# yutiansut/marl-optimal-execution

Hardware: AMD Instinct MI355X
Metric: env-steps/sec (whole node), rmsc03 100-agent market ×4096 envs, 1/2/4/8 GPUs (higher is better)
Workload: dtype int64; 1 GPU; rmsc03 x4096 envs per GPU, full episode per step (config build from seeds + the config's session), seeds 123456789+global_env; envs_per_gpu=4096, global_envs=4096, parallelism=envs sharded, dp1, parity_hash=False, env_errors=0, agents_per_env=64, device=AMD Radeon Graphics, cus=256

## Files before the change

include/mxa.h:

```cpp
#ifndef MXA_H
#define MXA_H
#include <stdint.h>
#ifdef __cplusplus
extern "C" {
#endif

typedef struct mxa_handle mxa_handle;

enum { MXA_RMSC03 = 0, MXA_SPARSE_ZI_100 = 1, MXA_SPARSE_ZI_1000 = 2, MXA_MARKETREPLAY = 3, MXA_RMSC03_RL = 4,
       MXA_VALUE_NOISE = 5 ,
       MXA_RMSC01 = 6 ,
       MXA_RMSC02 = 7 ,
       MXA_OBI_RMSC02 = 8 ,
       MXA_RANDOM_FUND_VALUE = 9 ,
       MXA_RANDOM_FUND_DIVERSE = 10 ,
       MXA_HIST_FUND_VALUE = 11 ,
       MXA_HIST_FUND_DIVERSE = 12 ,
       MXA_MARKETREPLAY_RUNNER = 13 ,
       MXA_MARKETREPLAY_TWAP = 14 ,
       MXA_RMSC03_SBMM = 15, MXA_RMSC03_SBMM_POLL = 16,
       MXA_RMSC03_MM = 17 };
enum {
  MXA_OK = 0, MXA_EINVAL = -1, MXA_EHIP = -2, MXA_ENOMEM = -3, MXA_ERANGE = -4
};
// ... 83 lines not shown
int mxa_set_launch_schedule(mxa_handle* h, int64_t first_chunk);
int mxa_set_stop_time(mxa_handle* h, int64_t t_stop_ns);
int mxa_run_until(mxa_handle* h, int64_t t_stop_ns, int64_t* events_out);
int mxa_finalize(mxa_handle* h);
int mxa_read_final(mxa_handle* h, int32_t env, mxa_agent_final* out, int32_t cap);
int mxa_read_summary(mxa_handle* h, mxa_env_summary* out );
int mxa_read_agents(mxa_handle* h, int32_t env, mxa_agent_state* out, int32_t cap);
int mxa_read_book(mxa_handle* h, int32_t env, int32_t side, int64_t* out4, int32_t cap);
int mxa_read_trace(mxa_handle* h, int32_t env, int64_t* out , int64_t cap, int64_t* n);
int mxa_set_seeds(mxa_handle* h, const uint32_t* seeds);
int mxa_write_results(mxa_handle* h, void* device_out);
#define MXA_RECORD_WORDS 12
int mxa_write_records(mxa_handle* h, void* device_out);
#define MXA_COUNTER_WORDS 34
int mxa_read_counters(mxa_handle* h, int64_t* out);
#define MXA_INPLACE_WORDS 6
int mxa_read_inplace(mxa_handle* h, uint64_t* out);
int mxa_read_raw(mxa_handle* h, int32_t env, int64_t offset, int64_t bytes, void* out);
int mxa_layout(const mxa_handle* h, int64_t* offsets8);
int32_t mxa_n_agents(const mxa_handle* h);
int32_t mxa_n_envs(const mxa_handle* h);
int64_t mxa_env_bytes(const mxa_handle* h);
int mxa_set_stream(mxa_handle* h, void* stream);
double mxa_last_kernel_ms(const mxa_handle* h);
const char* mxa_last_error(const mxa_handle* h);
void mxa_destroy(mxa_handle* h);

int mxa_create_replay(const int64_t* t, const int64_t* oid, const int64_t* price, const int64_t* size,
                      const int8_t* buy, int32_t n_rec, int32_t n_envs, int32_t device, int32_t trace_cap,
                      mxa_handle** out);
int mxa_create_replay_runner(const int64_t* t, const int64_t* oid, const int64_t* price, const int64_t* size,
// ... 26 lines not shown
  int32_t price;
  int32_t qty;
} mxa_book_rec;
#define MXA_BL_FUNDAMENTAL (-2147483647 - 1)
int mxa_set_book_log(mxa_handle* h, int32_t cap);
#define MXA_BL_EV_RX (-2147483647 - 1 + 256)
#define MXA_BL_EV_NT (MXA_BL_EV_RX + 256)
#define MXA_BL_EV_PLACE (MXA_BL_EV_RX + 512)
#define MXA_BL_EV_END (MXA_BL_EV_RX + 768)
int mxa_set_exchange_log(mxa_handle* h, int32_t on);
int mxa_read_book_log(mxa_handle* h, int32_t env, mxa_book_rec* out, int64_t cap, int64_t* n);

#include "mxa_snap.h"
#include "mxa_depth.h"
#include "mxa_bars.h"

int mxa_rng_probe(int32_t device, uint32_t seed, int32_t mode, double a, double b, int32_t n, double* out);
int mxa_math_probe(int32_t device, int32_t mode, const double* x, const double* y, double* out, int64_t n);
int mxa_policy_probe(void* stream, int32_t n, const float* x, const float* params, int32_t n_layers,
                     const int32_t* dims, int32_t test, int32_t enough, const double* u, const int64_t* rnd,
                     const double* eps, float* q, int64_t* a);

#ifdef __cplusplus
}
#endif
#endif
```

marl-optimal-execution_amd/build_lib.py:

```python
import hashlib
import os
import subprocess
import sys
from concurrent.futures import ThreadPoolExecutor

HERE = os.path.dirname(os.path.abspath(__file__))
ROOT = os.path.dirname(HERE)
SRC = os.path.join(HERE, "csrc", "mxa_api.hip")
INST = os.path.join(HERE, "csrc", "mxa_inst.hip")
OUT = os.path.join(HERE, "lib", "libmxa.so")
OBJ = os.path.join(HERE, "build")
N_CONFIGS = 18
DEPS = ["mxa_api.hip", "mxa_inst.hip", "mxa_entry.h", "mxa_kernels.hip", "mxa_layout.h", "mxa_config.h", "glibc_math.h",
        "glibc_math_tables.h", "qnet_wave_device.h", "ddqn_device.h", "mxa_snapshot.h", "mxa_depth_kernels.h",
        "mxa_bars_kernels.h"]
HIPCC = os.environ.get("HIPCC", "/opt/rocm/bin/hipcc")
FLAGS = ["--offload-arch=gfx950", "-O3", "-std=c++20", "-ffp-contract=off", "-fno-fast-math", "-fPIC", "-shared",
         "-Wno-unused-result", "-Wno-unused-value", "-mllvm", "-structurizecfg-skip-uniform-regions"]

CFG_FLAGS = {1: ["-mllvm", "-amdgpu-sched-strategy=max-ilp"], 2: ["-fno-slp-vectorize"],
             3: ["-mllvm", "-amdgpu-sched-strategy=max-ilp"]}


def sources():
    return [os.path.join(HERE, "csrc", d) for d in DEPS] + [os.path.join(ROOT, "include", h) for h in ("mxa.h", "mxa_snap.h", "mxa_depth.h", "mxa_bars.h")]


def build_id(extra=()):
    h = hashlib.sha256()
    for s in sources():
        with open(s, "rb") as f:
            h.update(f.read())
    h.update(" ".join(FLAGS + list(extra)).encode())
    h.update(repr(sorted(CFG_FLAGS.items())).encode())
    return h.hexdigest()[:16]


def up_to_date():
    if not os.path.exists(OUT):
        return False
# ... 54 lines not shown
```

marl-optimal-execution_amd/csrc/mxa_api.hip:

```cpp
#include <hip/hip_runtime.h>

#include <dlfcn.h>
#include <spawn.h>
#include <sys/stat.h>
#include <sys/wait.h>
#include <unistd.h>

#include <algorithm>
#include <cstddef>
#include <cstdio>
#include <cstdlib>
#include <cstring>
#include <map>
#include <memory>
#include <mutex>
#include <string>
#include <vector>

extern char** environ;

#include "../../include/mxa.h"
#define MXA_API_TU
#include "mxa_kernels.hip"
#include "mxa_entry.h"
// ... 1216 lines not shown
  hipSetDevice(h->device);
  delete h;
}

int mxa_rng_probe(int32_t device, uint32_t seed, int32_t mode, double a, double b, int32_t n, double* out) {
  if (n <= 0 || !out || mode < 0 || mode > 5) return MXA_EINVAL;
  if (hipSetDevice(device) != hipSuccess) return MXA_EHIP;
  DevBuf<double> d_out;
  DevBuf<uint32_t> d_s;
  if (d_out.alloc(n) != hipSuccess || d_s.alloc(MXA_RNG_WORDS) != hipSuccess) return MXA_ENOMEM;
  hipLaunchKernelGGL(mxa_rng_probe_kernel, dim3(1), dim3(64), 0, 0, seed, mode, a, b, n, d_out.p, d_s.p);
  if (hipGetLastError() != hipSuccess) return MXA_EHIP;
  return hipMemcpy(out, d_out, sizeof(double) * n, hipMemcpyDeviceToHost) == hipSuccess ? MXA_OK : MXA_EHIP;
}

int mxa_math_probe(int32_t device, int32_t mode, const double* x, const double* y, double* out, int64_t n) {
  if (n <= 0 || !x || !out) return MXA_EINVAL;
  if (hipSetDevice(device) != hipSuccess) return MXA_EHIP;
  DevBuf<double> dx, dy, dout;
  size_t bytes = sizeof(double) * n;
  if (dx.alloc(n) != hipSuccess || dy.alloc(n) != hipSuccess || dout.alloc(n) != hipSuccess) return MXA_ENOMEM;
  if (hipMemcpy(dx, x, bytes, hipMemcpyHostToDevice) != hipSuccess ||
      hipMemcpy(dy, y ? y : x, bytes, hipMemcpyHostToDevice) != hipSuccess)
    return MXA_EHIP;
  hipLaunchKernelGGL(mxa_math_probe_kernel, dim3((unsigned)((n + 255) / 256)), dim3(256), 0, 0, mode, dx.p, dy.p, dout.p,
                     n);
  if (hipGetLastError() != hipSuccess) return MXA_EHIP;
  return hipMemcpy(out, dout, bytes, hipMemcpyDeviceToHost) == hipSuccess ? MXA_OK : MXA_EHIP;
}

// ... 237 lines not shown
```

marl-optimal-execution_amd/csrc/mxa_config.h:

```cpp
#pragma once
#include <stddef.h>
#include "mxa_layout.h"
#include "../../include/mxa.h"

namespace mxa_cfg {

constexpr int64_t NS = 1000000000LL;
constexpr int64_t MIN = 60 * NS;
constexpr int64_t HOUR = 60 * MIN;

struct Shape {
  int sq, so;
  bool pl;
  int waves;
  int pw;
  int hot;
  int sql = 0;
};
constexpr int sq_lds(int cfg);
constexpr int lat_lds(int cfg);
constexpr Shape shape(int cfg);
#ifndef MXA_RMSC03_WAVES
#define MXA_RMSC03_WAVES 4
#endif
#ifndef MXA_RMSC01_WAVES
#define MXA_RMSC01_WAVES 4
#endif
#ifndef MXA_W_RMSC02
#define MXA_W_RMSC02 2
#endif
#ifndef MXA_BOOK_LDS_RMSC02
#define MXA_BOOK_LDS_RMSC02 0x34
#endif
#ifndef MXA_PL_RMSC02
#define MXA_PL_RMSC02 1
#endif
// ... 97 lines not shown
#define MXA_BOOK_LDS_RFV 0x34
#endif
constexpr int book_lds(int cfg) {
  return cfg == MXA_CFG_RMSC02 ? MXA_BOOK_LDS_RMSC02
         : (cfg >= MXA_CFG_RANDOM_FUND_VALUE && cfg <= MXA_CFG_HIST_FUND_DIVERSE) ? MXA_BOOK_LDS_RFV
                                                                                 : 0;
}
#ifndef MXA_TEMPER_FILL_MASK
#define MXA_TEMPER_FILL_MASK ((1 << MXA_CFG_RMSC03) | (1 << MXA_CFG_SPARSE_ZI_100) | (1 << MXA_CFG_VALUE_NOISE))
#endif
#ifndef MXA_ONE_ADVANCE_MASK
#define MXA_ONE_ADVANCE_MASK MXA_TEMPER_FILL_MASK
#endif
constexpr bool temper_fill(int cfg) { return (((MXA_TEMPER_FILL_MASK) >> cfg) & 1) != 0; }
constexpr bool one_advance(int cfg) { return (((MXA_ONE_ADVANCE_MASK) >> cfg) & 1) != 0; }
constexpr size_t lds_bytes(int cfg) {
  return (size_t)sq_lds(cfg) * 64 * (12 + (shape(cfg).pl ? 4 * shape(cfg).pw : 0)) + 512
         + (size_t)shape(cfg).hot * 512
         + 1024
         + (size_t)lat_lds(cfg) * 8
         + (rp_hdr_lds(cfg) ? 256 : 0)
         + (size_t)__builtin_popcount(book_lds(cfg)) * shape(cfg).so * 256
         + 256
#ifdef MXA_PROF
         + 1024
#endif
      ;
}

constexpr void base_params(MxaParams& P) {
  P.o_rbar = 1e5;
  P.o_kappa = 1.67e-12;
  P.o_fundvol = 1e-4;
  P.o_lambda = 2.77778e-13;
// ... 349 lines not shown
  off = align_up(off + (uint64_t)L.qcap * sizeof(SavedEvent) + (S.pl ? 0 : (uint64_t)L.qcap * 4 * S.pw) +
                     (uint64_t)(S.sq - sq_lds(cfg)) * 64 * 12,
                 256);
  L.off_book = (uint32_t)off;
  off = align_up(off + (uint64_t)L.ocap * sizeof(SavedOrder), 256);
  L.off_tx = (uint32_t)off;
  off = align_up(off + 64 + (uint64_t)L.tx_cap * sizeof(TxRec), 256);
  L.off_oh = off;
  off = align_up(off + (uint64_t)L.oh_cap * sizeof(OhRec), 256);
  L.off_hh = off;
  off = align_up(off + (uint64_t)L.hbl_range * 8, 256);
  L.off_sub = off;
  off = align_up(off + (P.md_sub ? (uint64_t)MD_MAX_SUBS * sizeof(SubRec) : 0), 256);
  L.off_md = off;
  off = align_up(off + (P.md_sub ? (uint64_t)P.n_agents * MD_WORDS * 4 : 0), 256);
  L.off_trace = (uint32_t)off;
  L.env_stride = off;
}

constexpr void params_value_noise(MxaParams& P) {
  base_params(P);
  P.config = MXA_CFG_VALUE_NOISE;
  P.ex_log_orders = 0;
  P.mkt_close = 10 * HOUR + 30 * MIN;
  P.start = 0;
  P.stop = 17 * HOUR;
  P.default_comp_delay = 1000000000;
  P.lat_mode = 1;
  P.noise_len = 6;
  P.lat_lo = 21000;
// ... 324 lines not shown
```

marl-optimal-execution_amd/csrc/mxa_kernels.hip:

```cpp
#pragma once
#include <hip/hip_runtime.h>
#if defined(MXA_ONLY_RMSC03) && !(defined(MXA_ONLY_CFG) && (MXA_ONLY_CFG == 3 || MXA_ONLY_CFG == 4))
#define MXA_NO_GYM
#endif

#ifndef MXA_HINT_MASK
#define MXA_HINT_MASK ((1 << 0) | (1 << 4))
#endif
#ifndef MXA_HINT_GROUPS
#define MXA_HINT_GROUPS 3
#endif
#if defined(MXA_INST_CFG)
#define MXA_HINT_ON (((MXA_HINT_MASK) >> (MXA_INST_CFG)) & 1)
#elif defined(MXA_ONLY_RMSC03) && defined(MXA_ONLY_CFG)
#define MXA_HINT_ON (((MXA_HINT_MASK) >> (MXA_ONLY_CFG)) & 1)
#elif defined(MXA_ONLY_RMSC03)
#define MXA_HINT_ON ((MXA_HINT_MASK) & 1)
#else
#define MXA_HINT_ON 0
#endif
#define MXA_EXPECT_(x, v) __builtin_expect(!!(x), v)
#define MXA_PROB_(x, v, p) __builtin_expect_with_probability(!!(x), v, p)
#if MXA_HINT_ON && ((MXA_HINT_GROUPS) & 1)
#define MXA_LIKELY(x) MXA_EXPECT_(x, 1)
// ... 337 lines not shown
    x1 = 2.0 * rs_double(r) - 1.0;
    x2 = 2.0 * rs_double(r) - 1.0;
    r2 = x1 * x1 + x2 * x2;
  } while (MXA_RARE_P(r2 >= 1.0 || r2 == 0.0, 0.215));
  f = __builtin_sqrt(-2.0 * gm_log(r2) / r2);
  r.gauss = f * x1;
  r.hasg |= 1;
  return f * x2;
}
template <bool B, int W, bool TF>
DEV double rs_normal(RSt<B, W, TF>& r, double loc, double scale) { return loc + scale * rs_gauss(r); }
template <bool B, int W, bool TF>
DEV double rs_exponential(RSt<B, W, TF>& r, double scale) { return scale * -gm_log(1.0 - rs_double(r)); }
template <bool B, int W, bool TF>
DEV double rs_uniform(RSt<B, W, TF>& r, double lo, double hi) { return lo + (hi - lo) * rs_double(r); }
template <int W, bool TF>
DEV void rs_skip_words(RSt<true, W, TF>& r, i64 k) {
  i64 target = (i64)r.p + k;
  while ((i64)r.m < target / MXA_MT_N) {
    mt_gen_build(r.key, r.m + 1);
    r.m++;
  }
  r.p = (i32)target;
}
#ifndef MXA_MAINT_LANES
#define MXA_MAINT_LANES 1
#endif
#ifndef MXA_WAKE_LANES
#define MXA_WAKE_LANES 1
#endif
// ... 243 lines not shown
  static constexpr int NG = QHIER ? (TIER_CFG ? mxa_cfg::sq_lds(CFG) / QG + 1 : SQ / QG) : 1;
  static constexpr bool QTREE = QHIER && QG >= 4;
  static constexpr int HOT = BUILD ? 0 : mxa_cfg::shape(CFG).hot;
  static constexpr bool RP = CFG == MXA_CFG_MARKETREPLAY || CFG == MXA_CFG_MARKETREPLAY_RUNNER ||
                             CFG == MXA_CFG_MARKETREPLAY_TWAP;
  static constexpr bool GYM = CFG == MXA_CFG_MARKETREPLAY || CFG == MXA_CFG_RMSC03_RL;
  static constexpr bool ACK_FAST = !BUILD && !RP && PC.default_comp_delay == 0 && PC.ex_comp == 0 &&
                                   PC.n_obi == 0;
  static constexpr bool RP_FAST = !BUILD && RP && PC.default_comp_delay == 0 && PC.ex_comp == 0;
  static constexpr int ACK_LIMIT = GYM ? PC.first_rl : PC.n_agents;
  static constexpr bool TFILL = MXA_TEMPER_AT_FILL != 0 && mxa_cfg::temper_fill(CFG);
  static constexpr bool ONE_ADV = MXA_ONE_ADVANCE != 0 && mxa_cfg::one_advance(CFG);
  typedef typename std::conditional<TFILL, RSt<BUILD, (!BUILD || MXA_BUILD_WINDOWS != 0) ? RS_WIN : RS_HBM, true>,
                                    RSt<BUILD>>::type RS;
  typedef typename std::conditional<BUILD || !TFILL, RS, RSt<false, RS_HBM, true>>::type ARS;
  typedef typename std::conditional<PL_LDS, LDSP u32*, u32*>::type PlPtr;
  static constexpr int QCAP = SQ * 64;
  static constexpr int KSH = MXA_KEY_SHIFT;
  static constexpr u64 KRCP = MXA_KEY_RCP;
  static_assert(PC.n_agents <= (int)KRCP, "recipient field of the event key");
  static constexpr int SQL = mxa_cfg::sq_lds(CFG);
  static constexpr bool TIER = SQL < SQ;
  static constexpr int QCL = SQL * 64;
  static_assert(!TIER || (!PL_LDS && SQL % 12 == 0 && SQ >= 16), "HBM queue tier: payloads in HBM, whole groups per tier");
  typedef typename std::conditional<TIER, GLBP char*, char*>::type EnvPtr;
  EnvPtr env;
  int lane;
  LDSP EnvHdr& h;
  i64 cur, pops, ocnt;
  i64 stop_t;
// ... 133 lines not shown
  i32 end_step;
  u32 run_skip;
  static constexpr bool BLOG = LOG;
  BlRec* blog;
  i32 blog_cap;
#ifdef MXA_PROF
  LDSP u64* prof;
#endif
  LDSP u64* hotrec;
  static constexpr int LATL = BUILD ? 0 : mxa_cfg::lat_lds(CFG);
  LDSP double* latl;
  static constexpr bool RPH = !BUILD && mxa_cfg::rp_hdr_lds(CFG);
  LDSP RpHdr* rhl;
  LDSP i32* scr;
  LDSP u32* rwin;

  static constexpr size_t LDS_Q = (size_t)QCL * (12 + (PL_LDS ? 4 * PW : 0));
  DEV Eng(char* e, char* lds, i32 tcap, const RpCtx* ctx = nullptr, BlRec* bl = nullptr, i32 bl_cap = 0)
      : env((EnvPtr)e), h(*(LDSP EnvHdr*)(lds + LDS_Q)) {
    rx = (const __attribute__((address_space(4))) RpCtx*)ctx;
    blog = bl;
    blog_cap = bl_cap;
    end_step = 0;
    add_delay = 0;
    run_skip = 0;
    rdirty = 0;
    lane = laneid();
    qk = (LDSP u64*)lds;
    qs = (LDSP u32*)(lds + 8 * QCL);
    if constexpr (PL_LDS) qpl = (LDSP u32*)(lds + 12 * QCL);
// ... 726 lines not shown
    else return PC.v_rbar;
  }
  DEV double v_sigma_n() {
    if constexpr (EXT) return rx->fs_v[0] / 10;
    else return PC.v_sigma_n;
  }

  DEV double o_compute(i64 ts, double v_adj, i64 pt, double pv) {
    i64 d = ts - pt;
    double mu = PC.o_rbar, gamma = PC.o_kappa, theta = PC.o_fundvol;
    const double ex = gm_exp(lane == 0 ? -gamma * (double)d : -2 * gamma * (double)d);
    double loc = mu + (pv - mu) * rdl_d(ex, 0);
    double scale = (h.o_th2 / (2 * gamma)) * (1 - rdl_d(ex, 1));
    (void)theta;
    RS O = grs(1);
    double v = rs_normal(O, loc, scale);
    grs_put(1, O);
    v += v_adj;
    if (!(v > 0)) v = 0;
    i64 vi = py_round(v);
    h.o_pt = ts;
    h.o_pv = (double)vi;
    if constexpr (BLOG) bl_put(ts, BL_FUNDAMENTAL, (i32)vi);
    return (double)vi;
  }
  DEV double o_advance(i64 t) {
    i64 pt = h.o_pt;
    double pv = h.o_pv;
    if (t <= pt) return pv;
    while (MXA_RARE(h.o_mst < t)) {
      double v = o_compute(h.o_mst, h.o_msv, pt, pv);
      pt = h.o_mst;
      pv = v;
      RS G = grs(0);
      h.o_mst = pt + (i64)rs_exponential(G, 1.0 / PC.o_lambda);
      grs_put(0, G);
      RS O = grs(1);
      double msv = rs_normal(O, PC.o_msmean, __builtin_sqrt(PC.o_msvar));
      h.o_msv = rs_randint(O, 0, 2) == 0 ? msv : -msv;
      grs_put(1, O);
    }
    return o_compute(t, 0, pt, pv);
  }
  DEV i64 o_observe(i64 t, double sigma_n) {
    PROF_SCOPE(69);
    if constexpr (EXT) {
      const double tp = efo_price(t);
      if (sigma_n == 0) return py_round(tp);
      ARS A = agent_rs();
      const i64 obs = py_round(rs_normal(A, tp, __builtin_sqrt(sigma_n)));
      agent_rs_put(A);
      return obs;
    }
    double r_t;
    if constexpr (ONE_ADV) r_t = o_advance(t >= PC.mkt_close ? PC.mkt_close - 1 : t);
    else r_t = t >= PC.mkt_close ? o_advance(PC.mkt_close - 1) : o_advance(t);
    if (sigma_n == 0) return (i64)r_t;
    ARS A = agent_rs();
    i64 obs = py_round(rs_normal(A, r_t, __builtin_sqrt(sigma_n)));
    agent_rs_put(A);
    return obs;
  }

  DEV i32 b_best(int buy_side) {
    PROF_SCOPE(68);
    i32 v = buy_side ? INT32_MIN : INT32_MAX;
    for (int j = 0; j < SO; j++) {
      bool m = bm[j] >= 0 && (bm[j] & 1) == buy_side;
      if (m) v = buy_side ? (bp[j] > v ? bp[j] : v) : (bp[j] < v ? bp[j] : v);
    }
    v = buy_side ? wmax_i32(v) : wmin_i32(v);
    return v;
  }
  DEV i64 b_level_qty(int buy_side, i32 price) {
// ... 978 lines not shown
  }

  DEV void value_wakeup() {
    if (!value_wake_head()) return;
    cancel_all();
    get_spread(1);
    rs(AF_STATE, AS_AWAITING_SPREAD);
  }
  DEV bool value_wake_head() {
    ta_wakeup();
    rs(AF_STATE, AS_INACTIVE);
    if (!fl(FL_HAS_OPEN) || !fl(FL_HAS_CLOSE)) return false;
    fl_set(FL_TRADING, true);
    if (fl(FL_MKT_CLOSED) && fl(FL_DAILY_CLOSE)) return false;
    ARS A = agent_rs();
    double dt = rs_exponential(A, 1.0 / PC.v_lambda);
    agent_rs_put(A);
    wakeup_at(cur_agent, cur + py_round(dt));
    if (fl(FL_MKT_CLOSED) && !fl(FL_DAILY_CLOSE)) {
      get_spread(1);
      rs(AF_STATE, AS_AWAITING_SPREAD);
      return false;
    }
    return true;
  }
  template <bool INPL = false>
  DEV int value_place(i64 room = 0) {
    i64 obs = o_observe(cur, v_sigma_n());
    i64 r_T = bayes_r_T(obs, PC.v_kappa, v_rbar(), v_sigma_n(), PC.v_sigma_s);
    i32 bid, ask;
    bool hb = known_bid(bid), ha = known_ask(ask);
    int buy;
    i64 p;
    RS G = grs(0);
    if (hb && ha) {
      i64 mid = (i64)((double)((i64)ask + bid) / 2);
      i64 spread = (i64)ask - bid;
      if (spread < 0) spread = -spread;
      i64 adj;
      if (rs_double(G) < PC.v_percent_aggr) adj = 0;
      else adj = rs_randint(G, 0, PC.v_depth_spread * spread);
      if (r_T < mid) {
        buy = 0;
// ... 1609 lines not shown
    const u64* src = (const u64*)hdr();
    u64* dst = (u64*)&h;
    if (lane < (int)(sizeof(EnvHdr) / 8)) dst[lane] = src[lane];
    wfence();
    cur = h.cur;
    stop_t = h.t_stop > 0 ? h.t_stop : PC.stop;
    pops = h.pops;
    ocnt = h.order_counter;
    hash = h.hash;
    seq = h.seq;
    status = h.status;
    err = h.err;
    qcount = h.q_count;
    maxq = h.max_q;
    if (lane < 4) h.rs_wn[lane] = 0;
    wfence();
    if constexpr (KREG) {
      kp = h.rs_pos[KS];
      km = h.rs_m[KS];
      khg = h.rs_has_gauss[KS];
      kw0 = h.rs_w0[KS];
      kwn = 0;
    }
  }
  DEV void hdr_to_global() {
    if (lane == 0) {
      h.cur = cur;
      h.pops = pops;
      h.order_counter = ocnt;
      h.hash = hash;
// ... 1152 lines not shown
    LDSP EnvHdr& h = this->h;
    i64 ocnt0 = 0;
    i32 tape_hi0 = 0;
    if (keep_ids) {
      ocnt0 = U(((const EnvHdr*)this->env)->order_counter);
      if constexpr (E::RP) {
        const RpHdr* R = this->rh();
        tape_hi0 = max(U(R->tape_hi), U(R->mr_done));
      }
    }
    {
      LDSP u32* hw = (LDSP u32*)&h;
      for (int i = this->lane; i < (int)(sizeof(EnvHdr) / 4); i += 64) hw[i] = 0;
      wfence();
    }
    this->hash = FNV_OFF;
    this->status = ST_RUNNING;
    this->err = 0;
    this->pops = 0;
    this->ocnt = ocnt0;
    this->seq = 0;
    this->qcount = 0;
    this->cur = P.start;
    for (int s = 0; s < 4; s++) {
      h.rs_pos[s] = MXA_MT_N;
      h.rs_m[s] = 0;
    }
    this->mk = KEY_EMPTY;
    this->ms = 0xFFFFFFFFu;
    this->mj = -1;
// ... 475 lines not shown
  r.hasg = 0;
  r.gauss = 0;
  for (int i = 0; i < n; i++) {
    double v;
    switch (mode) {
    case 0: v = (double)mxa::rs_u32(r); break;
    case 1: v = mxa::rs_double(r); break;
    case 2: v = (double)mxa::rs_randint(r, (int64_t)a, (int64_t)b); break;
    case 3: v = mxa::rs_normal(r, a, b); break;
    case 4: v = mxa::rs_exponential(r, a); break;
    default: v = mxa::rs_uniform(r, a, b); break;
    }
    if (__lane_id() == 0) out[i] = v;
  }
}
__global__ void mxa_math_probe_kernel(int mode, const double* x, const double* y, double* out, int64_t n) {
  int64_t i = (int64_t)blockIdx.x * blockDim.x + threadIdx.x;
  if (i >= n) return;
  out[i] = mode == 0 ? gm_log(x[i]) : mode == 1 ? gm_exp(x[i]) : gm_pow(x[i], y[i]);
}
struct MxaPolicyProbe {
  const float* params;
  int32_t n_layers, dims[qwave::kMaxLayers + 1];
  int32_t test, enough;
  const double* u;
  const int64_t* rnd;
  const double* eps;
};
__global__ __launch_bounds__(64) void mxa_policy_probe_kernel(MxaPolicyProbe p, int n, const float* x, float* q, int64_t* a) {
  const int row = blockIdx.x, lane = threadIdx.x;
// ... 18 lines not shown
```

marl-optimal-execution_amd/csrc/mxa_layout.h:

```cpp
#pragma once
#include <stdint.h>

#define MXA_MAX_AGENTS 8191
#define MXA_KEY_SHIFT 15
#define MXA_KEY_RCP 0x1FFF
#define MXA_MT_N 624
#define MXA_MT_M 397
#define MXA_RNG_WORDS 1280

enum mxa_config_id { MXA_CFG_RMSC03 = 0, MXA_CFG_SPARSE_ZI_100 = 1, MXA_CFG_SPARSE_ZI_1000 = 2, MXA_CFG_MARKETREPLAY = 3,
                     MXA_CFG_RMSC03_RL = 4, MXA_CFG_VALUE_NOISE = 5, MXA_CFG_RMSC01 = 6,
                     MXA_CFG_RMSC02 = 7, MXA_CFG_OBI_RMSC02 = 8, MXA_CFG_RANDOM_FUND_VALUE = 9,
                     MXA_CFG_RANDOM_FUND_DIVERSE = 10, MXA_CFG_HIST_FUND_VALUE = 11,
                     MXA_CFG_HIST_FUND_DIVERSE = 12, MXA_CFG_MARKETREPLAY_RUNNER = 13,
                     MXA_CFG_MARKETREPLAY_TWAP = 14,
                     MXA_CFG_RMSC03_SBMM = 15, MXA_CFG_RMSC03_SBMM_POLL = 16,
                     MXA_CFG_RMSC03_MM = 17 };

typedef struct {
  double pov;
  int32_t min_order_size;
  int32_t window_size;
  int32_t num_ticks;
  int32_t pad;
// ... 191 lines not shown
  const int64_t* fs_t;
  const double* fs_v;
  int32_t fs_n;
  int32_t twap_trade;
  RpLayout L;
  const MmParams* mmp;
} RpCtx;

typedef struct {
  uint64_t env_stride;
  uint32_t off_ag, off_open, off_rng, off_lat, off_q, off_book, off_tx, off_trace;
  int32_t n_agents, n_streams, qcap, ocap, open_cap, tx_cap, trace_cap, lat_len;
  int32_t oh_cap, hbl_range;
  uint64_t off_oh, off_hh;
  uint64_t off_sub, off_md;
} Layout;

#define MXA_AGENT_WORDS 128
#define MXA_AGENT_BYTES (MXA_AGENT_WORDS * 4)
enum {
  AF_TYPE = 0, AF_FLAGS = 1, AF_STATE = 2, AF_NORD = 3,
  AF_MKT_OPEN = 4, AF_MKT_CLOSE = 6, AF_CASH = 8, AF_SHARES = 10, AF_LAST_TRADE = 12,
  AF_BID = 14, AF_BIDQ = 15, AF_ASK = 16, AF_ASKQ = 17, AF_TV = 18, AF_PREV_WAKE = 20,
  AF_R_T = 22, AF_SIGMA_T = 24, AF_START_CASH = 26, AF_SIZE = 28, AF_GROUP = 29,
  AF_WAKEUP_TIME = 30, AF_RS_POS = 32, AF_RS_HASG = 33, AF_RS_GAUSS = 34, AF_LAST_MID = 36,
  AF_ORDER_SIZE = 38, AF_NMID = 39, AF_N20 = 40, AF_N50 = 41, AF_AVG20 = 42, AF_AVG50 = 44,
  AF_THETA = 46,
  AF_SB_N = 39, AF_SB_HEAD = 40, AF_SB_BLO = 41, AF_SB_ALO = 42, AF_SB_CNT = 43, AF_SB_IDS = 46,
  AF_MM_POV = AF_R_T, AF_MM_MIN = 46, AF_MM_WIN = 47, AF_MM_TICKS = 48, AF_MM_WAKE = 50,
  AF_MR_WI = 46, AF_MR_DONE = 47,
  AF_MIDS = 66,
  AF_STREAM_N = 66,
  AF_STREAM_HI = 68,
  AF_RS_M = 116,
  AF_NUSED = 117,
  AF_ATIME = 120,
  AF_COMP = 122,
  AF_END = MXA_AGENT_WORDS
};
enum {
  FL_HAS_OPEN = 1, FL_HAS_CLOSE = 2, FL_MKT_CLOSED = 4, FL_FIRST_WAKE = 8, FL_DAILY_CLOSE = 16,
  FL_TRADING = 32, FL_HAS_KNOWN = 64, FL_NB = 128, FL_NA = 256, FL_HAS_LAST = 512,
  FL_LAST_FLOAT = 1024, FL_PREV_WAKE = 2048, FL_AW_SPREAD = 4096, FL_AW_TV = 8192, FL_LAST_MID = 16384,
  FL_HAS_STREAM = 32768, FL_SUB_REQ = 65536,
  FL_OBI_LONG = 131072, FL_OBI_SHORT = 262144,
// ... 53 lines not shown
```

marl-optimal-execution_amd/mxabides/_lib.py:

```python
import ctypes
import os

PKG_ROOT = os.path.dirname(os.path.dirname(os.path.abspath(__file__)))
LIB_PATH = os.environ.get("MXA_LIB") or os.path.join(PKG_ROOT, "lib", "libmxa.so")

MXA_RMSC03, MXA_SPARSE_ZI_100, MXA_SPARSE_ZI_1000, MXA_MARKETREPLAY, MXA_RMSC03_RL, MXA_VALUE_NOISE = 0, 1, 2, 3, 4, 5
MXA_RMSC01 = 6
MXA_RMSC02 = 7
MXA_OBI_RMSC02 = 8
MXA_RANDOM_FUND_VALUE = 9
MXA_RANDOM_FUND_DIVERSE = 10
MXA_HIST_FUND_VALUE = 11
MXA_HIST_FUND_DIVERSE = 12
MXA_MARKETREPLAY_RUNNER = 13
MXA_MARKETREPLAY_TWAP = 14
MXA_RMSC03_SBMM = 15
MXA_RMSC03_SBMM_POLL = 16
MXA_RMSC03_MM = 17
CONFIG_IDS = {"rmsc03": MXA_RMSC03, "sparse_zi_100": MXA_SPARSE_ZI_100, "sparse_zi_1000": MXA_SPARSE_ZI_1000,
              "value_noise": MXA_VALUE_NOISE, "rmsc01": MXA_RMSC01, "rmsc02": MXA_RMSC02,
              "obi_rmsc02": MXA_OBI_RMSC02, "random_fund_value": MXA_RANDOM_FUND_VALUE,
              "random_fund_diverse": MXA_RANDOM_FUND_DIVERSE, "hist_fund_value": MXA_HIST_FUND_VALUE,
              "hist_fund_diverse": MXA_HIST_FUND_DIVERSE,
              "marketreplay_runner": MXA_MARKETREPLAY_RUNNER,
# ... 121 lines not shown
    "mxa_snapshot_create": ([_P, _I32, _OUT], _I32),
    "mxa_snapshot_save": ([_P, _P, _P], _I32),
    "mxa_snapshot_restore": ([_P, _P, _P], _I32),
    "mxa_snapshot_info": ([_P, _P], _I32),
    "mxa_snapshot_destroy": ([_P], None),
}
DEPTH_BINDINGS = {
    "mxa_write_depth": ([_P, _I32, _P, _P], _I32),
    "mxa_read_depth": ([_P, _I32, _P, _P], _I32),
}
BARS_BINDINGS = {
    "mxa_write_bars": ([_P, _I64, _I64, _I32, _P, _P], _I32),
    "mxa_read_bars": ([_P, _I64, _I64, _I32, _P, _P], _I32),
    "mxa_bars_from_records": ([_P, _I32, _P, _I64, _P, _I32, _I64, _I64, _I32, _P, _P], _I32),
}
COUNTER_WORDS = 34
INPLACE_WORDS = 6
RECORD_WORDS = 12

_lib = None


class MxaError(RuntimeError):
    pass


def load():
    global _lib
    if _lib is not None:
        return _lib
    if not os.path.exists(LIB_PATH):
        raise MxaError("libmxa.so not built (%s); run __graft_entry__.build()" % LIB_PATH)
    L = ctypes.CDLL(LIB_PATH)
    for name, (argtypes, restype) in list(BINDINGS.items()) + list(SNAPSHOT_BINDINGS.items()) + list(DEPTH_BINDINGS.items()) \
            + list(BARS_BINDINGS.items()):
        if hasattr(L, name):
            f = getattr(L, name)
            f.argtypes, f.restype = argtypes, restype
    _lib = L
    return L


def build_id():
    L = load()
    return L.mxa_build_id().decode() if hasattr(L, "mxa_build_id") else "unknown"
```

Before: 25.74 billion env-steps/s.

## Precompute wavefront-parallel gaussian/exponential variate tables for oracle and value agents

Adds lane-parallel variate tables: one wavefront fill tempers 128 Mersenne Twister words, converts them to uniforms, then computes polar-method gaussians and exponential logs for all lanes at once. The oracle's normal draws (table in LDS) and the value agents' noise and wakeup exponential draws (per-agent table in HBM) then read precomputed values instead of running the serial rejection/log path. Stream position and gauss caching stay consistent with the serial sampler, falling back to it when the table cannot serve a draw. The cost is extra LDS, per-agent HBM state, refill work on table misses, and added per-draw bookkeeping.

After: 27.02 billion env-steps/s, median of 6. 1.05x the previous value.

```diff
diff --git a/include/mxa.h b/include/mxa.h
--- a/include/mxa.h
+++ b/include/mxa.h
@@ -121,7 +121,7 @@
 int mxa_write_records(mxa_handle* h, void* device_out);
 #define MXA_COUNTER_WORDS 34
 int mxa_read_counters(mxa_handle* h, int64_t* out);
-#define MXA_INPLACE_WORDS 6
+#define MXA_INPLACE_WORDS 12
 int mxa_read_inplace(mxa_handle* h, uint64_t* out);
 int mxa_read_raw(mxa_handle* h, int32_t env, int64_t offset, int64_t bytes, void* out);
 int mxa_layout(const mxa_handle* h, int64_t* offsets8);
@@ -178,6 +178,7 @@
 #include "mxa_snap.h"
 #include "mxa_depth.h"
 #include "mxa_bars.h"
+#include "mxa_variates.h"
 
 int mxa_rng_probe(int32_t device, uint32_t seed, int32_t mode, double a, double b, int32_t n, double* out);
 int mxa_math_probe(int32_t device, int32_t mode, const double* x, const double* y, double* out, int64_t n);
diff --git a/include/mxa_variates.h b/include/mxa_variates.h
--- /dev/null
+++ b/include/mxa_variates.h
@@ -0,0 +1,14 @@
+#ifndef MXA_VARIATES_H
+#define MXA_VARIATES_H
+#include <stdint.h>
+#ifdef __cplusplus
+extern "C" {
+#endif
+
+int mxa_variate_probe(int32_t device, uint32_t seed, const uint8_t* script, int32_t n, int32_t lookahead, double* out,
+                      uint64_t* state);
+
+#ifdef __cplusplus
+}
+#endif
+#endif
diff --git a/marl-optimal-execution_amd/build_lib.py b/marl-optimal-execution_amd/build_lib.py
--- a/marl-optimal-execution_amd/build_lib.py
+++ b/marl-optimal-execution_amd/build_lib.py
@@ -23,7 +23,7 @@
 
 
 def sources():
-    return [os.path.join(HERE, "csrc", d) for d in DEPS] + [os.path.join(ROOT, "include", h) for h in ("mxa.h", "mxa_snap.h", "mxa_depth.h", "mxa_bars.h")]
+    return [os.path.join(HERE, "csrc", d) for d in DEPS] + [os.path.join(ROOT, "include", h) for h in ("mxa.h", "mxa_snap.h", "mxa_depth.h", "mxa_bars.h", "mxa_variates.h")]
 
 
 def build_id(extra=()):
diff --git a/marl-optimal-execution_amd/csrc/mxa_api.hip b/marl-optimal-execution_amd/csrc/mxa_api.hip
--- a/marl-optimal-execution_amd/csrc/mxa_api.hip
+++ b/marl-optimal-execution_amd/csrc/mxa_api.hip
@@ -1254,6 +1254,29 @@
   return hipMemcpy(out, d_out, sizeof(double) * n, hipMemcpyDeviceToHost) == hipSuccess ? MXA_OK : MXA_EHIP;
 }
 
+int mxa_variate_probe(int32_t device, uint32_t seed, const uint8_t* script, int32_t n, int32_t lookahead, double* out,
+                      uint64_t* state) {
+  if (n <= 0 || !script || !out || !state || lookahead < 2 || lookahead > 256) return MXA_EINVAL;
+  for (int32_t i = 0; i < n; i++)
+    if (script[i] > 3) return MXA_EINVAL;
+  if (hipSetDevice(device) != hipSuccess) return MXA_EHIP;
+  DevBuf<uint8_t> d_script;
+  DevBuf<double> d_out;
+  DevBuf<uint64_t> d_state, d_tab;
+  DevBuf<uint32_t> d_s;
+  if (d_script.alloc(n) != hipSuccess || d_out.alloc(2 * (size_t)n) != hipSuccess || d_state.alloc(6 * (size_t)n) != hipSuccess ||
+      d_tab.alloc(MXA_VT_BYTES / 8) != hipSuccess || d_s.alloc(2 * MXA_RNG_WORDS) != hipSuccess)
+    return MXA_ENOMEM;
+  if (hipMemcpy(d_script, script, (size_t)n, hipMemcpyHostToDevice) != hipSuccess ||
+      hipMemset(d_tab, 0, MXA_VT_BYTES) != hipSuccess)
+    return MXA_EHIP;
+  hipLaunchKernelGGL(mxa_variate_probe_kernel, dim3(1), dim3(64), 0, 0, seed, d_script.p, n, lookahead, d_out.p, d_state.p,
+                     d_s.p, d_tab.p);
+  if (hipGetLastError() != hipSuccess) return MXA_EHIP;
+  if (hipMemcpy(out, d_out, sizeof(double) * 2 * (size_t)n, hipMemcpyDeviceToHost) != hipSuccess) return MXA_EHIP;
+  return hipMemcpy(state, d_state, sizeof(uint64_t) * 6 * (size_t)n, hipMemcpyDeviceToHost) == hipSuccess ? MXA_OK : MXA_EHIP;
+}
+
 int mxa_math_probe(int32_t device, int32_t mode, const double* x, const double* y, double* out, int64_t n) {
   if (n <= 0 || !x || !out) return MXA_EINVAL;
   if (hipSetDevice(device) != hipSuccess) return MXA_EHIP;
diff --git a/marl-optimal-execution_amd/csrc/mxa_config.h b/marl-optimal-execution_amd/csrc/mxa_config.h
--- a/marl-optimal-execution_amd/csrc/mxa_config.h
+++ b/marl-optimal-execution_amd/csrc/mxa_config.h
@@ -20,6 +20,7 @@
 constexpr int sq_lds(int cfg);
 constexpr int lat_lds(int cfg);
 constexpr Shape shape(int cfg);
+constexpr bool is_custom(int cfg);
 #ifndef MXA_RMSC03_WAVES
 #define MXA_RMSC03_WAVES 4
 #endif
@@ -147,10 +148,26 @@
 #endif
 constexpr bool temper_fill(int cfg) { return (((MXA_TEMPER_FILL_MASK) >> cfg) & 1) != 0; }
 constexpr bool one_advance(int cfg) { return (((MXA_ONE_ADVANCE_MASK) >> cfg) & 1) != 0; }
+#ifndef MXA_VARIATE_TABLES
+#define MXA_VARIATE_TABLES 1
+#endif
+#ifndef MXA_VARIATE_O_MASK
+#define MXA_VARIATE_O_MASK (1 << MXA_CFG_RMSC03)
+#endif
+#ifndef MXA_VARIATE_AGENT_MASK
+#define MXA_VARIATE_AGENT_MASK (1 << MXA_CFG_RMSC03)
+#endif
+constexpr bool variate_o(int cfg) { return MXA_VARIATE_TABLES != 0 && (((MXA_VARIATE_O_MASK) >> cfg) & 1) != 0 && !is_custom(cfg); }
+constexpr bool variate_agent(int cfg) {
+  return MXA_VARIATE_TABLES != 0 && (((MXA_VARIATE_AGENT_MASK) >> cfg) & 1) != 0 && !is_custom(cfg);
+}
+#define MXA_VT_O_BYTES ((2 * 64 + 2) * 8)
+#define MXA_VT_BYTES 2048
 constexpr size_t lds_bytes(int cfg) {
   return (size_t)sq_lds(cfg) * 64 * (12 + (shape(cfg).pl ? 4 * shape(cfg).pw : 0)) + 512
          + (size_t)shape(cfg).hot * 512
          + 1024
+         + (variate_o(cfg) ? MXA_VT_O_BYTES : 0)
          + (size_t)lat_lds(cfg) * 8
          + (rp_hdr_lds(cfg) ? 256 : 0)
          + (size_t)__builtin_popcount(book_lds(cfg)) * shape(cfg).so * 256
@@ -530,6 +547,8 @@
   off = align_up(off + (P.md_sub ? (uint64_t)MD_MAX_SUBS * sizeof(SubRec) : 0), 256);
   L.off_md = off;
   off = align_up(off + (P.md_sub ? (uint64_t)P.n_agents * MD_WORDS * 4 : 0), 256);
+  L.off_vt = off;
+  off = align_up(off + (variate_agent(cfg) ? (uint64_t)P.n_value * MXA_VT_BYTES : 0), 256);
   L.off_trace = (uint32_t)off;
   L.env_stride = off;
 }
diff --git a/marl-optimal-execution_amd/csrc/mxa_kernels.hip b/marl-optimal-execution_amd/csrc/mxa_kernels.hip
--- a/marl-optimal-execution_amd/csrc/mxa_kernels.hip
+++ b/marl-optimal-execution_amd/csrc/mxa_kernels.hip
@@ -375,6 +375,104 @@
 DEV double rs_exponential(RSt<B, W, TF>& r, double scale) { return scale * -gm_log(1.0 - rs_double(r)); }
 template <bool B, int W, bool TF>
 DEV double rs_uniform(RSt<B, W, TF>& r, double lo, double hi) { return lo + (hi - lo) * rs_double(r); }
+struct VtDesc {
+  u64 acc;
+  i32 b, n;
+};
+template <bool EXP>
+struct VtIdx {
+  static constexpr int STRIDE = EXP ? 4 : 2, RET = EXP ? 1 : 0, CACHE = RET + 1;
+};
+DEV u64 vt_uni(u64 v) {
+  const u32 lo = (u32)__builtin_amdgcn_readfirstlane((i32)(u32)v), hi = (u32)__builtin_amdgcn_readfirstlane((i32)(u32)(v >> 32));
+  return ((u64)hi << 32) | lo;
+}
+template <bool EXP, class R, class T>
+DEV VtDesc vt_fill(const R& r, T tab, int cap = 128) {
+  typedef VtIdx<EXP> I;
+  const int lane = laneid();
+  const int q0 = r.p + 2 * lane, q1 = q0 + 1, b0 = q0 / MXA_MT_N, b1 = q1 / MXA_MT_N;
+  const bool ok = (cap >= 128 || 2 * lane + 1 < cap) && b0 >= r.m - 1 && b1 <= r.m;
+  u32 w0 = 0, w1 = 0;
+  if (ok) {
+    w0 = r.key[(b0 & 1) * MXA_MT_N + (q0 - b0 * MXA_MT_N)];
+    w1 = r.key[(b1 & 1) * MXA_MT_N + (q1 - b1 * MXA_MT_N)];
+  }
+  const i32 a = (i32)(mt_temper(w0) >> 5), b = (i32)(mt_temper(w1) >> 6);
+  const double u = ((double)a * 67108864.0 + (double)b) / 9007199254740992.0;
+  const u64 okb = bal(ok);
+  VtDesc d;
+  d.b = r.p;
+  d.n = ~okb == 0 ? 64 : ffs64(~okb);
+  if constexpr (EXP) {
+    tab[I::STRIDE * lane] = as_u(gm_log(1.0 - u));
+    tab[I::STRIDE * lane + 3] = 0;
+  }
+  const double x1 = 2.0 * u - 1.0;
+  const double x2 = __shfl_down(x1, 1, 64);
+  const double r2 = x1 * x1 + x2 * x2;
+  const bool acc = lane + 1 < d.n && !(r2 >= 1.0 || r2 == 0.0);
+  double f = 0.0;
+  if (acc) f = __builtin_sqrt(-2.0 * gm_log(r2) / r2);
+  tab[I::STRIDE * lane + I::RET] = as_u(acc ? f * x2 : 0.0);
+  tab[I::STRIDE * lane + I::CACHE] = as_u(acc ? f * x1 : 0.0);
+  d.acc = bal(acc);
+  wfence();
+  return d;
+}
+template <class R, class T>
+DEV bool vt_exp(R& r, T tab, const VtDesc& d, double& e) {
+  const u32 off = (u32)(r.p - d.b);
+  if ((off & 1u) || (off >> 1) >= (u32)d.n) return false;
+  e = as_d(vt_uni(tab[VtIdx<true>::STRIDE * (off >> 1)]));
+  r.p += 2;
+  return true;
+}
+template <bool EXP, class R, class T>
+DEV bool vt_gauss(R& r, T tab, const VtDesc& d, double& g) {
+  typedef VtIdx<EXP> I;
+  const u32 off = (u32)(r.p - d.b), i = off >> 1;
+  if ((off & 1u) || i + 1 >= (u32)d.n) return false;
+  const u64 m = d.acc & (0x5555555555555555ull << (i & 1u)) & (~0ull << i);
+  if (!m) return false;
+  const int j = ctz64(m);
+  g = as_d(vt_uni(tab[I::STRIDE * j + I::RET]));
+  r.gauss = as_d(vt_uni(tab[I::STRIDE * j + I::CACHE]));
+  r.hasg |= 1;
+  r.p = d.b + 2 * j + 4;
+  return true;
+}
+template <bool EXP, class R, class T, class P, class C>
+DEV double vt_draw_gauss(R& r, T tab, VtDesc d, P put, C count, int cap = 128) {
+  if (r.hasg & 1) return rs_gauss_serial(r);
+  double g;
+  if (MXA_RARE(!vt_gauss<EXP>(r, tab, d, g))) {
+    d = vt_fill<EXP>(r, tab, cap);
+    put(d);
+    count(1);
+    if (!vt_gauss<EXP>(r, tab, d, g)) {
+      count(2);
+      return rs_gauss_serial(r);
+    }
+  }
+  count(0);
+  return g;
+}
+template <class R, class T, class P, class C>
+DEV double vt_draw_exponential(R& r, T tab, VtDesc d, double scale, P put, C count, int cap = 128) {
+  double e;
+  if (MXA_RARE(!vt_exp(r, tab, d, e))) {
+    d = vt_fill<true>(r, tab, cap);
+    put(d);
+    count(1);
+    if (!vt_exp(r, tab, d, e)) {
+      count(2);
+      return rs_exponential(r, scale);
+    }
+  }
+  count(0);
+  return scale * -e;
+}
 template <int W, bool TF>
 DEV void rs_skip_words(RSt<true, W, TF>& r, i64 k) {
   i64 target = (i64)r.p + k;
@@ -648,6 +746,8 @@
   typedef typename std::conditional<TFILL, RSt<BUILD, (!BUILD || MXA_BUILD_WINDOWS != 0) ? RS_WIN : RS_HBM, true>,
                                     RSt<BUILD>>::type RS;
   typedef typename std::conditional<BUILD || !TFILL, RS, RSt<false, RS_HBM, true>>::type ARS;
+  static constexpr bool VT_O = !BUILD && mxa_cfg::variate_o(CFG);
+  static constexpr bool VT_A = !BUILD && mxa_cfg::variate_agent(CFG) && PC.n_value > 0;
   typedef typename std::conditional<PL_LDS, LDSP u32*, u32*>::type PlPtr;
   static constexpr int QCAP = SQ * 64;
   static constexpr int KSH = MXA_KEY_SHIFT;
@@ -811,6 +911,40 @@
   LDSP RpHdr* rhl;
   LDSP i32* scr;
   LDSP u32* rwin;
+  DEV LDSP u64* otab() { return (LDSP u64*)((LDSP char*)rwin - MXA_VT_O_BYTES); }
+  DEV VtDesc odesc() {
+    const u64 bn = vt_uni(otab()[129]);
+    return VtDesc{vt_uni(otab()[128]), (i32)(u32)bn, (i32)(u32)(bn >> 32)};
+  }
+  DEV void odesc_put(const VtDesc& d) {
+    if (lane == 0) {
+      otab()[128] = d.acc;
+      otab()[129] = (u64)(u32)d.b | ((u64)(u32)d.n << 32);
+    }
+    wfence();
+  }
+  DEV u64* atab() { return (u64*)(env + PC.L.off_vt + (size_t)(cur_agent - PC.first_value) * MXA_VT_BYTES); }
+  DEV VtDesc adesc() { return VtDesc{(u64)rg64(AF_VT_ACC), rgi(AF_VT_B), rgi(AF_VT_N)}; }
+  DEV void adesc_put(const VtDesc& d) {
+    rs(AF_VT_B, (u32)d.b);
+    rs(AF_VT_N, (u32)d.n);
+    rs64(AF_VT_ACC, (i64)d.acc);
+  }
+  template <int USER>
+  DEV void vt_count(int what) {
+    if constexpr (INSTR && !BUILD) {
+      if ((hash_on || trace) && lane == 0) atomicAdd(&g_mxa_inplace[6 + 3 * USER + what], 1ull);
+    }
+  }
+  DEV double o_normal(RS& O, double loc, double scale) {
+    if constexpr (VT_O) return loc + scale * vt_draw_gauss<false>(O, otab(), odesc(), [&](const VtDesc& d) { odesc_put(d); }, [&](int w) { vt_count<0>(w); });
+    else return rs_normal(O, loc, scale);
+  }
+  template <bool VAL>
+  DEV double agent_normal(ARS& A, double loc, double scale) {
+    if constexpr (VAL && VT_A) return loc + scale * vt_draw_gauss<true>(A, atab(), adesc(), [&](const VtDesc& d) { adesc_put(d); }, [&](int w) { vt_count<1>(w); });
+    else return rs_normal(A, loc, scale);
+  }
 
   static constexpr size_t LDS_Q = (size_t)QCL * (12 + (PL_LDS ? 4 * PW : 0));
   DEV Eng(char* e, char* lds, i32 tcap, const RpCtx* ctx = nullptr, BlRec* bl = nullptr, i32 bl_cap = 0)
@@ -1567,7 +1701,7 @@
     double scale = (h.o_th2 / (2 * gamma)) * (1 - rdl_d(ex, 1));
     (void)theta;
     RS O = grs(1);
-    double v = rs_normal(O, loc, scale);
+    double v = o_normal(O, loc, scale);
     grs_put(1, O);
     v += v_adj;
     if (!(v > 0)) v = 0;
@@ -1589,19 +1723,20 @@
       h.o_mst = pt + (i64)rs_exponential(G, 1.0 / PC.o_lambda);
       grs_put(0, G);
       RS O = grs(1);
-      double msv = rs_normal(O, PC.o_msmean, __builtin_sqrt(PC.o_msvar));
+      double msv = o_normal(O, PC.o_msmean, __builtin_sqrt(PC.o_msvar));
       h.o_msv = rs_randint(O, 0, 2) == 0 ? msv : -msv;
       grs_put(1, O);
     }
     return o_compute(t, 0, pt, pv);
   }
+  template <bool VAL = false>
   DEV i64 o_observe(i64 t, double sigma_n) {
     PROF_SCOPE(69);
     if constexpr (EXT) {
       const double tp = efo_price(t);
       if (sigma_n == 0) return py_round(tp);
       ARS A = agent_rs();
-      const i64 obs = py_round(rs_normal(A, tp, __builtin_sqrt(sigma_n)));
+      const i64 obs = py_round(agent_normal<VAL>(A, tp, __builtin_sqrt(sigma_n)));
       agent_rs_put(A);
       return obs;
     }
@@ -1610,7 +1745,7 @@
     else r_t = t >= PC.mkt_close ? o_advance(PC.mkt_close - 1) : o_advance(t);
     if (sigma_n == 0) return (i64)r_t;
     ARS A = agent_rs();
-    i64 obs = py_round(rs_normal(A, r_t, __builtin_sqrt(sigma_n)));
+    i64 obs = py_round(agent_normal<VAL>(A, r_t, __builtin_sqrt(sigma_n)));
     agent_rs_put(A);
     return obs;
   }
@@ -2619,7 +2754,9 @@
     fl_set(FL_TRADING, true);
     if (fl(FL_MKT_CLOSED) && fl(FL_DAILY_CLOSE)) return false;
     ARS A = agent_rs();
-    double dt = rs_exponential(A, 1.0 / PC.v_lambda);
+    double dt;
+    if constexpr (VT_A) dt = vt_draw_exponential(A, atab(), adesc(), 1.0 / PC.v_lambda, [&](const VtDesc& d) { adesc_put(d); }, [&](int w) { vt_count<1>(w); });
+    else dt = rs_exponential(A, 1.0 / PC.v_lambda);
     agent_rs_put(A);
     wakeup_at(cur_agent, cur + py_round(dt));
     if (fl(FL_MKT_CLOSED) && !fl(FL_DAILY_CLOSE)) {
@@ -2631,7 +2768,7 @@
   }
   template <bool INPL = false>
   DEV int value_place(i64 room = 0) {
-    i64 obs = o_observe(cur, v_sigma_n());
+    i64 obs = o_observe<true>(cur, v_sigma_n());
     i64 r_T = bayes_r_T(obs, PC.v_kappa, v_rbar(), v_sigma_n(), PC.v_sigma_s);
     i32 bid, ask;
     bool hb = known_bid(bid), ha = known_ask(ask);
@@ -4271,6 +4408,8 @@
     qcount = h.q_count;
     maxq = h.max_q;
     if (lane < 4) h.rs_wn[lane] = 0;
+    if constexpr (VT_O)
+      if (lane == 0) otab()[129] = 0;
     wfence();
     if constexpr (KREG) {
       kp = h.rs_pos[KS];
@@ -5453,6 +5592,10 @@
       for (int i = this->lane; i < (int)(sizeof(EnvHdr) / 4); i += 64) hw[i] = 0;
       wfence();
     }
+    if constexpr (mxa_cfg::variate_agent(CFG) && E::PC.n_value > 0) {
+      u64* vt = (u64*)(this->env + P.L.off_vt);
+      for (int i = this->lane; i < P.n_value * (MXA_VT_BYTES / 8); i += 64) vt[i] = 0;
+    }
     this->hash = FNV_OFF;
     this->status = ST_RUNNING;
     this->err = 0;
@@ -5958,6 +6101,39 @@
     if (__lane_id() == 0) out[i] = v;
   }
 }
+__global__ __launch_bounds__(64) void mxa_variate_probe_kernel(uint32_t seed, const uint8_t* script, int n, int cap, double* out,
+                                                               uint64_t* state, uint32_t* scratch, uint64_t* tab) {
+  for (int pass = 0; pass < 2; pass++) {
+    mxa::RSt<true> r;
+    r.lw = nullptr;
+    r.lw0 = r.lwn = 0;
+    r.key = scratch + pass * MXA_RNG_WORDS;
+    mxa::mt_seed(r.key, seed);
+    r.p = MXA_MT_N;
+    r.m = 0;
+    r.hasg = 0;
+    r.gauss = 0;
+    auto none = [](int) {};
+    mxa::VtDesc d{0, 0, 0};
+    auto put = [&](const mxa::VtDesc& x) { d = x; };
+    for (int i = 0; i < n; i++) {
+      const int kind = script[i];
+      double v;
+      if (pass == 0) mxa::rs_maint(r, MXA_AGENT_LA);
+      if (kind == 0) v = pass == 0 ? mxa::vt_draw_exponential(r, tab, d, 1.0, put, none, cap) : mxa::rs_exponential(r, 1.0);
+      else if (kind == 1) v = pass == 0 ? mxa::vt_draw_gauss<true>(r, tab, d, put, none, cap) : mxa::rs_gauss_serial(r);
+      else if (kind == 2) v = (double)mxa::rs_u32(r);
+      else v = (double)mxa::rs_randint(r, 0, 100);
+      if (__lane_id() == 0) {
+        const size_t k = (size_t)pass * n + i;
+        out[k] = v;
+        state[3 * k] = (uint64_t)(uint32_t)r.p;
+        state[3 * k + 1] = (uint64_t)(uint32_t)r.hasg;
+        state[3 * k + 2] = mxa::as_u(r.gauss);
+      }
+    }
+  }
+}
 __global__ void mxa_math_probe_kernel(int mode, const double* x, const double* y, double* out, int64_t n) {
   int64_t i = (int64_t)blockIdx.x * blockDim.x + threadIdx.x;
   if (i >= n) return;
diff --git a/marl-optimal-execution_amd/csrc/mxa_layout.h b/marl-optimal-execution_amd/csrc/mxa_layout.h
--- a/marl-optimal-execution_amd/csrc/mxa_layout.h
+++ b/marl-optimal-execution_amd/csrc/mxa_layout.h
@@ -229,6 +229,7 @@
   int32_t oh_cap, hbl_range;
   uint64_t off_oh, off_hh;
   uint64_t off_sub, off_md;
+  uint64_t off_vt;
 } Layout;
 
 #define MXA_AGENT_WORDS 128
@@ -244,6 +245,7 @@
   AF_SB_N = 39, AF_SB_HEAD = 40, AF_SB_BLO = 41, AF_SB_ALO = 42, AF_SB_CNT = 43, AF_SB_IDS = 46,
   AF_MM_POV = AF_R_T, AF_MM_MIN = 46, AF_MM_WIN = 47, AF_MM_TICKS = 48, AF_MM_WAKE = 50,
   AF_MR_WI = 46, AF_MR_DONE = 47,
+  AF_VT_B = 46, AF_VT_N = 47, AF_VT_ACC = 48,
   AF_MIDS = 66,
   AF_STREAM_N = 66,
   AF_STREAM_HI = 68,
diff --git a/marl-optimal-execution_amd/mxabides/_lib.py b/marl-optimal-execution_amd/mxabides/_lib.py
--- a/marl-optimal-execution_amd/mxabides/_lib.py
+++ b/marl-optimal-execution_amd/mxabides/_lib.py
@@ -159,8 +159,11 @@
     "mxa_read_bars": ([_P, _I64, _I64, _I32, _P, _P], _I32),
     "mxa_bars_from_records": ([_P, _I32, _P, _I64, _P, _I32, _I64, _I64, _I32, _P, _P], _I32),
 }
+VARIATE_BINDINGS = {
+    "mxa_variate_probe": ([_I32, _U32, _P, _I32, _I32, _P, _P], _I32),
+}
 COUNTER_WORDS = 34
-INPLACE_WORDS = 6
+INPLACE_WORDS = 12
 RECORD_WORDS = 12
 
 _lib = None
@@ -178,7 +181,7 @@
         raise MxaError("libmxa.so not built (%s); run __graft_entry__.build()" % LIB_PATH)
     L = ctypes.CDLL(LIB_PATH)
     for name, (argtypes, restype) in list(BINDINGS.items()) + list(SNAPSHOT_BINDINGS.items()) + list(DEPTH_BINDINGS.items()) \
-            + list(BARS_BINDINGS.items()):
+            + list(BARS_BINDINGS.items()) + list(VARIATE_BINDINGS.items()):
         if hasattr(L, name):
             f = getattr(L, name)
             f.argtypes, f.restype = argtypes, restype
```
